# PFLeget/treegp

Hardware: AMD Instinct MI355X
Metric: GP solve+predict throughput, 2-D AnisotropicRBF N=65536 (higher is better)
Workload: dtype f64

## Files before the change

include/tgp.h:

```cpp
#ifndef TGP_H
#define TGP_H

#include <stdint.h>

#ifdef __cplusplus
extern "C" {
#endif

typedef struct tgp_ctx tgp_ctx;
typedef struct tgp_factor tgp_factor;

enum {
    TGP_RBF = 0,
    TGP_ARBF = 1,
    TGP_VK = 2,
    TGP_AVK = 3
};

typedef struct {
    int32_t kind;
    int32_t _pad;
    double amp;
    double a, b, c;
    double ell;
// ... 202 lines not shown
int tgp_d_kbuild_lower(tgp_ctx *ctx, const tgp_kernel *k, const double *d_X, int64_t n,
                       const double *d_yerr, double *d_A);
int tgp_d_potrf(tgp_ctx *ctx, double *d_A, int64_t Np, double *d_W);
int tgp_d_potrs(tgp_ctx *ctx, const double *d_A, const double *d_W, int64_t Np, double *d_b);
int tgp_d_potrs_multi(tgp_ctx *ctx, const double *d_A, const double *d_W, int64_t Np, double *d_B, int nrhs);
int tgp_d_unpack_lower(tgp_ctx *ctx, const double *d_A, int64_t Np, int64_t n, double *out);
int tgp_factor_device(tgp_ctx *ctx, const tgp_factor *f, const double **d_A, const double **d_W, int64_t *Np);
int tgp_set_stream(tgp_ctx *ctx, void *hip_stream);
int tgp_reset_stream(tgp_ctx *ctx);
int tgp_set_side_stream(tgp_ctx *ctx, void *hip_stream);
int64_t tgp_dist_panel_rows(int64_t p, int64_t Np, int G, int g);
int64_t tgp_dist_panel_off(int64_t p, int64_t Np, int G, int g);
int64_t tgp_dist_local_elems(int64_t Np, int G, int g);
int tgp_dd_kbuild(tgp_ctx *ctx, const tgp_kernel *k, const double *d_X, int64_t n, const double *d_yerr,
                  double *d_Aloc, const int64_t *d_loff, int G, int g);
int tgp_dd_factor_diag(tgp_ctx *ctx, double *d_Aloc, const int64_t *h_loff, int64_t Np, int kpanel, int G, int g,
                       double *d_W, double *d_bcast);
int tgp_dd_trsm(tgp_ctx *ctx, double *d_Aloc, const int64_t *h_loff, int64_t Np, int kpanel, int G, int g,
                double *d_W, const double *d_bcast);
int tgp_dd_update(tgp_ctx *ctx, double *d_Aloc, const int64_t *d_loff, int64_t Np, int kpanel, int G, int g,
                  const double *d_gathered, int cmax, int col_lo, int col_hi);
int tgp_dd_update2(tgp_ctx *ctx, double *d_Aloc, const int64_t *d_loff, int64_t Np, int kpanel, int G, int g,
                   const double *d_gathered0, int cmax0, const double *d_gathered1, int cmax1, int col_lo,
                   int col_hi);
int tgp_dd_update_group(tgp_ctx *ctx, double *d_Aloc, const int64_t *d_loff, int64_t Np, int kpanel, int G, int g,
                        int nseg, const double *const *d_gathered, const int *cmax, int col_lo, int col_hi);
int tgp_dd_strip_left(tgp_ctx *ctx, double *d_Aloc, const int64_t *h_loff, const int64_t *d_loff, int64_t Np, int kgroup, int b,
                      int G, int g, const double *d_ext);
int tgp_dd_queue_reset(tgp_ctx *ctx);
int tgp_dd_set_exclusive(tgp_ctx *ctx, int on);
int tgp_dd_update_group_queued(tgp_ctx *ctx, double *d_Aloc, const int64_t *d_loff, int64_t Np, int kpanel, int G, int g,
                               int nseg, const double *const *d_gathered, const int *cmax, int col_lo, int col_hi, int nres);
int tgp_dd_update_group_fused(tgp_ctx *ctx, double *d_Aloc, const int64_t *d_loff, int64_t Np, int kpanel, int G, int g, int nseg,
                              const double *const *d_gathered, const int *cmax, int head_cols, int nres);
int tgp_dd_wait_head(tgp_ctx *ctx, tgp_ctx *waiter);
int tgp_dd_tail_assemble(tgp_ctx *ctx, const double *d_gathered, int64_t stride, int64_t Np, int k0, int G, double *d_tail);
int tgp_dd_tail_scatter(tgp_ctx *ctx, const double *d_tail, int64_t Np, int k0, int G, int g, double *d_Aloc, const int64_t *d_loff);
int tgp_handoff_mode(tgp_ctx *ctx);
int tgp_dd_keep_panel(tgp_ctx *ctx, double *d_Afull, int64_t Np, int kpanel, int G, const double *d_bcast,
                      const double *d_gathered, int cmax);
int tgp_dd_fwd_diag(tgp_ctx *ctx, const double *d_Aloc, const int64_t *h_loff, int kb, const double *d_W, double *d_yk);
int tgp_dd_fwd_update(tgp_ctx *ctx, const double *d_Aloc, const int64_t *h_loff, int64_t Np, int kb, int G, int g,
                      const double *d_zk, double *d_yloc);
int tgp_dd_bwd_partial(tgp_ctx *ctx, const double *d_Aloc, const int64_t *h_loff, int64_t Np, int kb, int G, int g,
                       const double *d_aloc, double *d_s);
int tgp_dd_bwd_diag(tgp_ctx *ctx, const double *d_Aloc, const int64_t *h_loff, int kb, const double *d_W, double *d_ak,
                    const double *d_s );
int tgp_dd_logdet_local(tgp_ctx *ctx, const double *d_Aloc, const int64_t *d_loff, int64_t Np, int64_t n, int G, int g,
                        double *d_out);
int tgp_dd_info(tgp_ctx *ctx, int reset);

int tgp_debug_syrk_loop(tgp_ctx *ctx, double *d_A, int64_t Np, int reps, double *ms_per_launch,
                        double *flops_per_launch);
int tgp_debug_tilemap(int64_t T, int32_t *ti, int32_t *tj, int64_t cap);

#ifdef __cplusplus
}
#endif
#endif
```

treegp_amd/_lib.py:

```python
import ctypes as C
import os
import threading

import numpy as np

_HERE = os.path.dirname(os.path.abspath(__file__))
LIB_PATH = os.environ.get("TGP_LIB_PATH") or os.path.join(_HERE, "csrc", "libtgp.so")

TGP_RBF, TGP_ARBF, TGP_VK, TGP_AVK = 0, 1, 2, 3
NTIMINGS = 12


class TgpKernel(C.Structure):
    _fields_ = [("kind", C.c_int32), ("_pad", C.c_int32), ("amp", C.c_double), ("a", C.c_double),
                ("b", C.c_double), ("c", C.c_double), ("ell", C.c_double)]


TGP_SUM_MAX = 4


class TgpKernelSum(C.Structure):
    _fields_ = [("nterms", C.c_int32), ("_pad", C.c_int32), ("term", TgpKernel * TGP_SUM_MAX)]


# ... 43 lines not shown
    "tgp_d_gp_predict": (C.c_int, [_vp, C.POINTER(TgpKernel), _vp, _i64, _vp, _vp, _i64, _vp]),
    "tgp_d_gp_predict_grad": (C.c_int, [_vp, C.POINTER(TgpKernel), _vp, _i64, _vp, _vp, _i64, _vp]),
    "tgp_panel_off": (_i64, [_i64, _i64]),
    "tgp_panel_elems": (_i64, [_i64]),
    "tgp_padded_n": (_i64, [_i64]),
    "tgp_d_kbuild_lower": (C.c_int, [_vp, C.POINTER(TgpKernel), _vp, _i64, _vp, _vp]),
    "tgp_d_potrf": (C.c_int, [_vp, _vp, _i64, _vp]),
    "tgp_d_potrs": (C.c_int, [_vp, _vp, _vp, _i64, _vp]),
    "tgp_d_potrs_multi": (C.c_int, [_vp, _vp, _vp, _i64, _vp, C.c_int]),
    "tgp_gp_solve_dense": (C.c_int, [_vp, _vp, _i64, _vp, _vp, _vp, _dp, _dp, C.POINTER(_vp)]),
    "tgp_d_gp_solve_dense": (C.c_int, [_vp, _vp, _i64, _vp, _vp, _vp, _dp, _dp, C.POINTER(_vp)]),
    "tgp_factor_solve": (C.c_int, [_vp, _vp, _vp, C.c_int, _vp]),
    "tgp_factor_lmul": (C.c_int, [_vp, _vp, _vp, C.c_int, _vp]),
    "tgp_factor_inv_diag": (C.c_int, [_vp, _vp, _vp]),
    "tgp_factor_inv_blocks": (C.c_int, [_vp, _vp, _vp, _i64, _vp]),
    "tgp_gp_solve_batch": (C.c_int, [_vp, C.c_int, _vp, _vp, _i64, _vp, _vp, _vp, _vp, _vp, _vp, _vp]),
    "tgp_gp_solve_grad_batch": (C.c_int, [_vp, C.c_int, _vp, _vp, _i64, _vp, _vp, _vp, _vp, _vp, _vp, _vp]),
    "tgp_gp_loo_batch": (C.c_int, [_vp, C.c_int, _vp, _vp, _i64, _vp, _vp, _vp, _vp, _vp, _vp, _vp, _vp]),
    "tgp_gp_posterior_batch": (C.c_int, [_vp, C.c_int, _vp, _vp, _i64, _vp, _vp, _vp, _vp, _i64, _vp, C.c_int, _vp, _vp, _vp, _vp, _vp]),
    "tgp_gp_predict_cov_dense": (C.c_int, [_vp, _vp, _vp, _vp, _i64, _vp]),
    "tgp_gp_predict_var": (C.c_int, [_vp, _vp, C.POINTER(TgpKernel), _vp, _i64, _vp, _i64, _vp]),
    "tgp_gp_predict_var_dense": (C.c_int, [_vp, _vp, _vp, _vp, _i64, _vp]),
    "tgp_gp_loglik_grad": (C.c_int, [_vp, _vp, C.POINTER(TgpKernel), _vp, _i64, _vp, _vp]),
    "tgp_d_gp_solve_grad": (C.c_int, [_vp, C.POINTER(TgpKernel), _vp, _i64, _vp, _vp, _dp, _dp, _vp]),
    "tgp_gp_loglik_grad_any": (C.c_int, [_vp, _vp, C.POINTER(TgpKernel), _vp, _i64, _vp, _vp]),
    "tgp_d_gp_solve_grad_any": (C.c_int, [_vp, C.POINTER(TgpKernel), _vp, _i64, _vp, _vp, _dp, _dp, _vp]),
    "tgp_gp_solve_grad_batch_any": (C.c_int, [_vp, C.c_int, _vp, _vp, _i64, _vp, _vp, _vp, _vp, _vp, _vp, _vp]),
    "tgp_kernel_matrix_sum": (C.c_int, [_vp, C.POINTER(TgpKernelSum), _vp, _i64, _vp, _i64, _vp]),
    "tgp_d_kbuild_lower_sum": (C.c_int, [_vp, C.POINTER(TgpKernelSum), _vp, _i64, _vp, _vp]),
    "tgp_gp_solve_sum": (C.c_int, [_vp, C.POINTER(TgpKernelSum), _vp, _i64, _vp, _vp, _vp, _dp, _dp, C.POINTER(_vp)]),
    "tgp_gp_predict_sum": (C.c_int, [_vp, C.POINTER(TgpKernelSum), _vp, _i64, _vp, _vp, _i64, _vp]),
    "tgp_gp_predict_grad_sum": (C.c_int, [_vp, C.POINTER(TgpKernelSum), _vp, _i64, _vp, _vp, _i64, _vp]),
    "tgp_gp_predict_cov_sum": (C.c_int, [_vp, _vp, C.POINTER(TgpKernelSum), _vp, _i64, _vp, _i64, _vp]),
    "tgp_gp_predict_var_sum": (C.c_int, [_vp, _vp, C.POINTER(TgpKernelSum), _vp, _i64, _vp, _i64, _vp]),
    "tgp_gp_loglik_grad_sum": (C.c_int, [_vp, _vp, C.POINTER(TgpKernelSum), _vp, _i64, _vp, _vp]),
    "tgp_gp_fisher": (C.c_int, [_vp, _vp, C.POINTER(TgpKernel), _vp, _i64, _vp]),
    "tgp_gp_fisher_sum": (C.c_int, [_vp, _vp, C.POINTER(TgpKernelSum), _vp, _i64, _vp]),
    "tgp_gp_solve_batch_sum": (C.c_int, [_vp, C.c_int, C.POINTER(TgpKernelSum), _vp, _i64, _vp, _vp, _vp, _vp, _vp, _vp, _vp]),
    "tgp_gp_posterior_batch_sum": (C.c_int, [_vp, C.c_int, C.POINTER(TgpKernelSum), _vp, _i64, _vp, _vp, _vp, _vp, _i64, _vp, C.c_int,
                                             _vp, _vp, _vp, _vp, _vp]),
    "tgp_gp_loo_batch_sum": (C.c_int, [_vp, C.c_int, C.POINTER(TgpKernelSum), _vp, _i64, _vp, _vp, _vp, _vp, _vp, _vp, _vp, _vp]),
    "tgp_gp_solve_grad_batch_sum": (C.c_int, [_vp, C.c_int, C.POINTER(TgpKernelSum), _vp, _i64, _vp, _vp, _vp, _vp, _vp, _vp, _vp]),
    "tgp_kbuild_batch_sum": (C.c_int, [_vp, C.c_int, C.POINTER(TgpKernelSum), _vp, _i64, _vp, _vp, _vp]),
    "tgp_kernel_matrix3": (C.c_int, [_vp, C.POINTER(TgpKernel3), _vp, _i64, _vp, _i64, _vp]),
    "tgp_d_kbuild_lower3": (C.c_int, [_vp, C.POINTER(TgpKernel3), _vp, _i64, _vp, _vp]),
    "tgp_gp_solve3": (C.c_int, [_vp, C.POINTER(TgpKernel3), _vp, _i64, _vp, _vp, _vp, _dp, _dp, C.POINTER(_vp)]),
    "tgp_gp_predict3": (C.c_int, [_vp, C.POINTER(TgpKernel3), _vp, _i64, _vp, _vp, _i64, _vp]),
    "tgp_gp_predict_grad3": (C.c_int, [_vp, C.POINTER(TgpKernel3), _vp, _i64, _vp, _vp, _i64, _vp]),
    "tgp_gp_predict_cov3": (C.c_int, [_vp, _vp, C.POINTER(TgpKernel3), _vp, _i64, _vp, _i64, _vp]),
    "tgp_gp_predict_var3": (C.c_int, [_vp, _vp, C.POINTER(TgpKernel3), _vp, _i64, _vp, _i64, _vp]),
    "tgp_d_unpack_lower":(C.c_int, [_vp, _vp, _i64, _i64, _vp]),
    "tgp_factor_device": (C.c_int, [_vp, _vp, C.POINTER(_vp), C.POINTER(_vp), C.POINTER(_i64)]),
    "tgp_debug_syrk_loop": (C.c_int, [_vp, _vp, _i64, C.c_int, _dp, _dp]),
    "tgp_debug_tilemap": (C.c_int, [_i64, _vp, _vp, _i64]),
    "tgp_set_stream": (C.c_int, [_vp, _vp]),
    "tgp_reset_stream": (C.c_int, [_vp]),
    "tgp_set_side_stream": (C.c_int, [_vp, _vp]),
    "tgp_dist_panel_rows": (_i64, [_i64, _i64, C.c_int, C.c_int]),
    "tgp_dist_panel_off": (_i64, [_i64, _i64, C.c_int, C.c_int]),
    "tgp_dist_local_elems": (_i64, [_i64, C.c_int, C.c_int]),
    "tgp_dd_kbuild": (C.c_int, [_vp, C.POINTER(TgpKernel), _vp, _i64, _vp, _vp, _vp, C.c_int, C.c_int]),
    "tgp_dd_factor_diag": (C.c_int, [_vp, _vp, _vp, _i64, C.c_int, C.c_int, C.c_int, _vp, _vp]),
    "tgp_dd_trsm": (C.c_int, [_vp, _vp, _vp, _i64, C.c_int, C.c_int, C.c_int, _vp, _vp]),
    "tgp_dd_update": (C.c_int, [_vp, _vp, _vp, _i64, C.c_int, C.c_int, C.c_int, _vp, C.c_int, C.c_int, C.c_int]),
    "tgp_dd_update2": (C.c_int, [_vp, _vp, _vp, _i64, C.c_int, C.c_int, C.c_int, _vp, C.c_int, _vp, C.c_int, C.c_int, C.c_int]),
    "tgp_dd_update_group": (C.c_int, [_vp, _vp, _vp, _i64, C.c_int, C.c_int, C.c_int, C.c_int, _vp, _vp, C.c_int, C.c_int]),
    "tgp_dd_strip_left": (C.c_int, [_vp, _vp, _vp, _vp, _i64, C.c_int, C.c_int, C.c_int, C.c_int, _vp]),
    "tgp_dd_update_group_queued": (C.c_int, [_vp, _vp, _vp, _i64, C.c_int, C.c_int, C.c_int, C.c_int, _vp, _vp, C.c_int, C.c_int, C.c_int]),
    "tgp_dd_update_group_fused": (C.c_int, [_vp, _vp, _vp, _i64, C.c_int, C.c_int, C.c_int, C.c_int, _vp, _vp, C.c_int, C.c_int]),
    "tgp_dd_wait_head": (C.c_int, [_vp, _vp]),
    "tgp_handoff_mode": (C.c_int, [_vp]),
    "tgp_dd_tail_assemble": (C.c_int, [_vp, _vp, _i64, _i64, C.c_int, C.c_int, _vp]),
    "tgp_dd_tail_scatter": (C.c_int, [_vp, _vp, _i64, C.c_int, C.c_int, C.c_int, _vp, _vp]),
    "tgp_dd_queue_reset": (C.c_int, [_vp]),
    "tgp_dd_set_exclusive": (C.c_int, [_vp, C.c_int]),
    "tgp_dd_keep_panel": (C.c_int, [_vp, _vp, _i64, C.c_int, C.c_int, _vp, _vp, C.c_int]),
    "tgp_dd_fwd_diag": (C.c_int, [_vp, _vp, _vp, C.c_int, _vp, _vp]),
    "tgp_dd_fwd_update": (C.c_int, [_vp, _vp, _vp, _i64, C.c_int, C.c_int, C.c_int, _vp, _vp]),
    "tgp_dd_bwd_partial": (C.c_int, [_vp, _vp, _vp, _i64, C.c_int, C.c_int, C.c_int, _vp, _vp]),
    "tgp_dd_bwd_diag": (C.c_int, [_vp, _vp, _vp, C.c_int, _vp, _vp, _vp]),
    "tgp_dd_logdet_local": (C.c_int, [_vp, _vp, _vp, _i64, _i64, C.c_int, C.c_int, _vp]),
    "tgp_dd_info": (C.c_int, [_vp, C.c_int]),
}

_lib = None
_ctx = {}
_lock = threading.Lock()


def _share_hip_runtime_with_torch():
    import sys
    if "torch" in sys.modules or os.environ.get("TGP_SYSTEM_HIP") == "1":
        return
    try:
        import importlib.util
        spec = importlib.util.find_spec("torch")
        if spec is None or not spec.origin:
            return
        cand = os.path.join(os.path.dirname(spec.origin), "lib", "libamdhip64.so")
        if os.path.exists(cand):
            C.CDLL(cand, mode=C.RTLD_GLOBAL)
            if os.environ.get("TGP_VERBOSE"):
                print("treegp_amd: using torch's HIP runtime %s (one HIP runtime per process)" % cand, file=sys.stderr)
    except Exception:
        pass

# ... 123 lines not shown
```

treegp_amd/csrc/chol.hip:

```cpp
#include "tgp_internal.h"

#include "gemm_tile.h"
#include "potrf128.h"

#ifdef TGP_POTRF_STAMPS
__device__ unsigned long long tgp_gemm_stamps[1024 * 4];
__device__ int tgp_gemm_stamp_grid = 43;
__device__ unsigned long long tgp_queue_stamps[1024 * 4];
__device__ int tgp_queue_stamp_T = 40;
__device__ unsigned long long tgp_mid_stamps[25 * 8];
__device__ int tgp_mid_stamp_base = 5120;
#define TGP_MID_STAMP(i)                                                                                   \
    do {                                                                                                   \
        if (threadIdx.x == 0 && base == tgp_mid_stamp_base && blockIdx.x < 25) tgp_mid_stamps[blockIdx.x * 8 + (i)] = __builtin_amdgcn_s_memrealtime(); \
    } while (0)
#else
#define TGP_MID_STAMP(i) ((void)0)
#endif

namespace {
template <int MODE, int LDB>
__global__ __launch_bounds__(256, 2) void gemm_col_kernel(const double *A, const double *B, double *C) {
    const int64_t t = blockIdx.x;
    TGP_CHAIN_PRIO();
#ifdef TGP_POTRF_STAMPS
    const unsigned long long t_in = __builtin_amdgcn_s_memrealtime();
#endif
    gemm_tile_128<MODE, LDB, TGP_TB>(A + t * 128 * TGP_PW, B, C + t * 128 * TGP_PW);
#ifdef TGP_POTRF_STAMPS
    if (MODE == 0 && threadIdx.x == 0 && (int)gridDim.x == tgp_gemm_stamp_grid) {
        tgp_gemm_stamps[blockIdx.x * 4 + 0] = t_in;
        tgp_gemm_stamps[blockIdx.x * 4 + 1] = __builtin_amdgcn_s_memrealtime();
        tgp_gemm_stamps[blockIdx.x * 4 + 2] = (__builtin_amdgcn_s_getreg(20 | (0 << 6) | (3 << 11)) << 8) | __builtin_amdgcn_s_getreg(4 | (8 << 6) | (7 << 11));
    }
#endif
}

template <int MODE, int LDB>
__global__ __launch_bounds__(256) void gemm_col_small_kernel(const double *A, const double *B, double *C) {
    const int64_t o = (int64_t)blockIdx.x * 16 * TGP_PW;
    TGP_CHAIN_PRIO();
    nt_slice_tile<MODE, TGP_TB, 1>(nt_slice_lds_storage(), A + o, TGP_PW, B, LDB, C + o, TGP_PW, nullptr, nullptr);
}
__device__ __forceinline__ void keep_w_share(double *__restrict__ keep, const double *__restrict__ W0) {
    if (!keep) return;
    constexpr int n2 = TGP_TB * TGP_TB;
    const int per = (n2 + (int)gridDim.x - 1) / (int)gridDim.x;
    const int lo = (int)blockIdx.x * per, hi = lo + per < n2 ? lo + per : n2;
    for (int i = lo + (int)threadIdx.x; i < hi; i += 256)
        reinterpret_cast<double2 *>(keep)[i] = reinterpret_cast<const double2 *>(W0)[i];
}
__global__ __launch_bounds__(256, 2) void panel_tall_kernel(double *rows0, const double *W0, const double *L10, const double *W1,
                                                            double *keep) {
    double *rows = rows0 + (int64_t)blockIdx.x * 128 * TGP_PW;
    TGP_CHAIN_PRIO();
    keep_w_share(keep, W0);
    gemm_tile_128<0, TGP_TB, TGP_TB>(rows, W0, rows);
    __syncthreads();
    gemm_tile_128<1, TGP_PW, TGP_TB>(rows, L10, rows + TGP_TB);
    __syncthreads();
    gemm_tile_128<0, TGP_TB, TGP_TB>(rows + TGP_TB, W1, rows + TGP_TB);
}

__global__ __launch_bounds__(256) void panel_tall_small_kernel(double *rows0, const double *W0, const double *L10, const double *W1,
                                                               double *keep) {
    double *rows = rows0 + (int64_t)blockIdx.x * 16 * TGP_PW;
    TGP_CHAIN_PRIO();
    keep_w_share(keep, W0);
    double *lds = nt_slice_lds_storage();
    nt_slice_tile<0, TGP_TB, 1>(lds, rows, TGP_PW, W0, TGP_TB, rows, TGP_PW, nullptr, nullptr);
    asm volatile("s_waitcnt vmcnt(0)" ::: "memory");
    __syncthreads();
    nt_slice_tile<1, TGP_TB, 1>(lds, rows, TGP_PW, L10, TGP_PW, rows + TGP_TB, TGP_PW, nullptr, nullptr);
    asm volatile("s_waitcnt vmcnt(0)" ::: "memory");
    __syncthreads();
    nt_slice_tile<0, TGP_TB, 1>(lds, rows + TGP_TB, TGP_PW, W1, TGP_TB, rows + TGP_TB, TGP_PW, nullptr, nullptr);
}

__global__ __launch_bounds__(256, 2) void diag_mid_kernel(double *R1, const double *W0) {
    TGP_CHAIN_PRIO();
    gemm_tile_128<0, TGP_TB, TGP_TB>(R1, W0, R1);
    __syncthreads();
    gemm_tile_128<1, TGP_PW, TGP_TB>(R1, R1, R1 + TGP_TB);
}

constexpr unsigned long long PANEL_SPIN_TICKS = 5000000ull;
constexpr int PANEL_SYNC_WORDS = 16;
__device__ __forceinline__ void panel_publish(unsigned *counter) {
    asm volatile("s_waitcnt vmcnt(0)" ::: "memory");
    __syncthreads();
    if (threadIdx.x == 0) {
        __builtin_amdgcn_fence(__ATOMIC_RELEASE, "agent");
        __hip_atomic_fetch_add(counter, 1u, __ATOMIC_RELAXED, __HIP_MEMORY_SCOPE_AGENT);
    }
}
__device__ __forceinline__ bool panel_wait(unsigned *sync, int which, unsigned target, int *info) {
    __shared__ int s_ok;
    if (threadIdx.x == 0) {
        int ok = 1;
        const unsigned long long t0 = __builtin_amdgcn_s_memrealtime();
        unsigned it = 0;
        while (__hip_atomic_load(sync + which, __ATOMIC_RELAXED, __HIP_MEMORY_SCOPE_AGENT) < target) {
            __builtin_amdgcn_s_sleep(1);
            if ((++it & 63u) == 0u) {
                const bool late = __builtin_amdgcn_s_memrealtime() - t0 > PANEL_SPIN_TICKS;
                if (late || __hip_atomic_load(sync + 2, __ATOMIC_RELAXED, __HIP_MEMORY_SCOPE_AGENT) != 0u) {
                    __hip_atomic_store(sync + 2, 1u, __ATOMIC_RELAXED, __HIP_MEMORY_SCOPE_AGENT);
                    if (late) __hip_atomic_store(info, -7, __ATOMIC_RELAXED, __HIP_MEMORY_SCOPE_AGENT);
                    ok = 0;
                    break;
                }
            }
        }
        __builtin_amdgcn_fence(__ATOMIC_ACQUIRE, "agent");
// ... 360 lines not shown

template <int NSEG>
__global__ __launch_bounds__(256, 2) void syrk_distn_queue_kernel(double *Aloc, const int64_t *__restrict__ loff, int kpanel, int G,
                                                                  int g, DistSegs<NSEG> S, int col_lo, int ncol, int nrows, DistMap M,
                                                                  unsigned slots_per_class, int nres, unsigned *__restrict__ queue) {
    __shared__ unsigned s_slot;
    const unsigned xcd = blockIdx.x & 7;
    if (threadIdx.x == 0) {
        const unsigned hw = __builtin_amdgcn_s_getreg(4 | (8 << 6) | (7 << 11));
        const unsigned xcc = __builtin_amdgcn_s_getreg(20 | (0 << 6) | (3 << 11)) & 7;
        const unsigned key = hw + 1;
        unsigned *claims = queue + 8 + TGP_QUEUE_MAXRES * (4 * xcc + ((hw >> 5) & 3));
        unsigned leave = 0;
        for (int r = 0; r < nres && !leave; ++r) {
            const unsigned prev = atomicCAS(&claims[r], 0u, key);
            leave = (prev == 0u || prev == key) ? 1u : 0u;
        }
        if (leave && atomicAdd(&queue[TGP_QUEUE_LEAVE + xcd], 1u) >= 8u * (unsigned)nres + 8u) leave = 0u;
        s_slot = leave;
    }
    __syncthreads();
    const bool leave = s_slot != 0u;
    __syncthreads();
    if (leave) return;
    for (;;) {
        if (threadIdx.x == 0) s_slot = atomicAdd(&queue[xcd], 1u);
        __syncthreads();
        const unsigned n = s_slot;
        __syncthreads();
        if (n >= slots_per_class) break;
        syrk_distn_tile<NSEG>(((int64_t)n << 3) | xcd, Aloc, loff, kpanel, G, g, S, col_lo, ncol, nrows, M);
        __syncthreads();
    }
}

inline void run_potrf128(hipStream_t st, double *A, int lda, double *W, int *info, int base, bool exclusive = false, bool solo = false) {
    constexpr unsigned image = potrf_v2::POTRF_LDS_BYTES, full = 128 * 1024;
    static const bool attr_ok = [] {
        return hipFuncSetAttribute((const void *)potrf_v2::potrf128_kernel<true>, hipFuncAttributeMaxDynamicSharedMemorySize, (int)full) == hipSuccess &&
               hipFuncSetAttribute((const void *)potrf_v2::potrf128_solo_kernel, hipFuncAttributeMaxDynamicSharedMemorySize, (int)full) == hipSuccess;
    }();
    (void)attr_ok;
    if (exclusive || solo) potrf_v2::potrf128_solo_kernel<<<1, 256, exclusive ? full : image, st>>>(A, lda, W, info, base);
    else potrf_v2::potrf128_kernel<true><<<1, 256, image, st>>>(A, lda, W, info, base);
}
}

namespace {
__global__ void set_identity128_kernel(double *__restrict__ W) {
    const int t = blockIdx.x * 256 + threadIdx.x;
    W[t] = (t >> 7) == (t & 127) ? 1.0 : 0.0;
}

void factor_panel(hipStream_t st, double *Pk, int64_t mk, double *W0, int *d_info, int base, bool exclusive = false,
                  int64_t n_data = -1, unsigned *mid_sync = nullptr, int cu_budget = 0) {
    double *W1 = W0 + TGP_TB * TGP_TB;
    double *R1 = Pk + (int64_t)TGP_TB * TGP_PW;
    const int r1 = (int)((mk - TGP_TB) / TGP_TB);
    static const int small_rows = [] { const char *e = getenv("TGP_SMALL_ROWS"); return e ? atoi(e) : 80; }();
    const bool solo = cu_budget >= 256 && mid_sync != nullptr;
    run_potrf128(st, Pk, TGP_PW, W0, d_info, base, exclusive, solo);
    if (n_data >= 0 && (int64_t)base + TGP_TB >= n_data && mk == TGP_PW) {
        gemm_col_small_kernel<0, TGP_TB><<<8, 256, 0, st>>>(R1, W0, R1);
        set_identity128_kernel<<<64, 256, 0, st>>>(W1);
        return;
    }
    const int r2 = (int)((mk - TGP_PW) / TGP_TB);
    if (mid_sync) {
        constexpr unsigned pad = 128 * 1024 - potrf_v2::POTRF_LDS_DOUBLES * 8;
        static const bool pad_ok = [] {
            return hipFuncSetAttribute((const void *)panel_mid_kernel<true>, hipFuncAttributeMaxDynamicSharedMemorySize, (int)pad) == hipSuccess &&
                   hipFuncSetAttribute((const void *)panel_mid_kernel<false>, hipFuncAttributeMaxDynamicSharedMemorySize, (int)pad) == hipSuccess;
        }();
        const unsigned dyn = (exclusive && pad_ok) ? pad : 0u;
        if (17 + 8 * r2 <= cu_budget) panel_mid_kernel<true><<<25 + 8 * r2, 256, dyn, st>>>(Pk, W0, W1, d_info, base, mid_sync);
        else panel_mid_kernel<false><<<25 + r2, 256, dyn, st>>>(Pk, W0, W1, d_info, base, mid_sync);
    } else if (cu_budget > 0) {
        double *R2 = Pk + (int64_t)TGP_PW * TGP_PW;
        const bool small = 17 + 8 * r2 <= cu_budget;
        gemm_col_small_kernel<0, TGP_TB><<<8, 256, 0, st>>>(R1, W0, R1);
        if (r2 > 0) {
            if (small) gemm_col_small_kernel<0, TGP_TB><<<r2 * 8, 256, 0, st>>>(R2, W0, R2);
            else gemm_col_kernel<0, TGP_TB><<<r2, 256, 0, st>>>(R2, W0, R2);
        }
        gemm_col_small_kernel<1, TGP_PW><<<8, 256, 0, st>>>(R1, R1, R1 + TGP_TB);
        if (r2 > 0) {
            if (small) gemm_col_small_kernel<1, TGP_PW><<<r2 * 8, 256, 0, st>>>(R2, R1, R2 + TGP_TB);
            else gemm_col_kernel<1, TGP_PW><<<r2, 256, 0, st>>>(R2, R1, R2 + TGP_TB);
        }
        run_potrf128(st, R1 + TGP_TB, TGP_PW, W1, d_info, base + TGP_TB, exclusive, solo);
    } else {
        if (r1 <= small_rows) {
            gemm_col_small_kernel<0, TGP_TB><<<r1 * 8, 256, 0, st>>>(R1, W0, R1);
            gemm_col_small_kernel<1, TGP_PW><<<r1 * 8, 256, 0, st>>>(R1, R1, R1 + TGP_TB);
        } else {
            gemm_col_kernel<0, TGP_TB><<<r1, 256, 0, st>>>(R1, W0, R1);
            gemm_col_kernel<1, TGP_PW><<<r1, 256, 0, st>>>(R1, R1, R1 + TGP_TB);
        }
        run_potrf128(st, R1 + TGP_TB, TGP_PW, W1, d_info, base + TGP_TB, exclusive, solo);
    }
    if (r2 > 0) {
        double *R2 = Pk + (int64_t)TGP_PW * TGP_PW + TGP_TB;
        if (r2 <= small_rows) gemm_col_small_kernel<0, TGP_TB><<<r2 * 8, 256, 0, st>>>(R2, W1, R2);
        else gemm_col_kernel<0, TGP_TB><<<r2, 256, 0, st>>>(R2, W1, R2);
    }
}

inline int diag_full() {
    static const int v = [] { const char *e = getenv("TGP_DIAG_FULL"); return e ? (atoi(e) != 0 ? 1 : 0) : 0; }();
    return v;
}

inline int small_t() {
    static const int v = [] { const char *e = getenv("TGP_SMALL_T"); return e ? atoi(e) : 8; }();
    return v;
}

template <int NSEG>
void launch_syrk(hipStream_t st, double *d_A, int64_t Np, int ob, int T, int strip, const double *P0, const double *P1) {
    if (T <= 0) return;
    static const int strip_small_t = [] { const char *e = getenv("TGP_STRIP_SMALL_T"); return e ? atoi(e) : 16; }();
    if (T <= small_t() || (strip > 0 && T <= strip_small_t)) {
        const int cols = strip == 0 ? T : (strip < T ? strip : T);
        syrk_small_kernel<NSEG><<<dim3((unsigned)(T * 8), (unsigned)cols), 256, 0, st>>>(d_A, Np, ob, T, P0, P1);
        return;
    }
    static const int strip64_t = [] { const char *e = getenv("TGP_STRIP64_T"); return e ? atoi(e) : 128; }();
    static const int strip32_t = [] { const char *e = getenv("TGP_STRIP32_T"); return e ? atoi(e) : 64; }();
    if (strip > 0 && T <= strip32_t) {
        syrk_strip32_kernel<NSEG><<<(unsigned)((int64_t)4 * T * strip), 256, 0, st>>>(d_A, Np, ob, T, strip, P0, P1);
        return;
    }
    if (strip > 0 && T <= strip64_t) {
        syrk_strip64_kernel<NSEG><<<(unsigned)((int64_t)2 * T * strip), 256, 0, st>>>(d_A, Np, ob, T, strip, P0, P1);
        return;
    }
    const unsigned gs = strip == 0 ? (unsigned)tilemap_grid(T) : (unsigned)((int64_t)T * strip);
    syrk_dtv_kernel<NSEG><<<gs, 256, 0, st>>>(d_A, Np, ob, T, strip, P0, P1, diag_full());
}

int queued_nres(int T) {
    static const int queue_res = [] { const char *e = getenv("TGP_QUEUE_RES"); return e ? atoi(e) : 0; }();
    if (queue_res > 0) return queue_res > TGP_QUEUE_MAXRES ? TGP_QUEUE_MAXRES : queue_res;
    static const int t1 = [] { const char *e = getenv("TGP_QUEUE_T1"); return e ? atoi(e) : 42; }();
    static const int t2 = [] { const char *e = getenv("TGP_QUEUE_T2"); return e ? atoi(e) : 26; }();
    return T >= t1 ? 1 : (T >= t2 ? 2 : 3);
}
void launch_syrk2_queued(tgp_ctx *ctx, hipStream_t st, double *d_A, int64_t Np, int ob, int T, const double *P0, const double *P1,
                         int nqueue) {
    const int nres = queued_nres(T);
    static const int half_env = [] { const char *e = getenv("TGP_QUEUE_HALF"); return e ? atoi(e) : -1; }();
    const unsigned slots = (unsigned)(tilemap_grid(T) / 8);
    unsigned nhalf = half_env >= 0 ? (unsigned)half_env : (unsigned)(512 - 64 * nres) / 8u;
    if (nhalf > slots) nhalf = slots;
    static const int steal = [] { const char *e = getenv("TGP_QUEUE_STEAL"); return e ? atoi(e) : 1; }();
    syrk_dtv_queue_kernel<2><<<512 + 8, 256, 0, st>>>(d_A, Np, ob, T, slots + nhalf, slots - nhalf, nres,
// ... 207 lines not shown
            }
        }
    }
    TGP_HIP(hipGetLastError());
    TGP_HIP(hipMemcpyAsync(ctx->h_info, ctx->d_info, sizeof(int), hipMemcpyDeviceToHost, st));
    ctx->timings[6] = nlaunch;
    ctx->timings[7] = flops;
    ctx->timings[5] = 0.0;
    if (defer_info && !prof) return 0;
    TGP_HIP(hipStreamSynchronize(st));
    if (prof) {
        double tot = 0.0;
        for (int i = 0; i < nlaunch; ++i) {
            float ms = 0.f;
            TGP_HIP(hipEventElapsedTime(&ms, ctx->prof_events[2 * i], ctx->prof_events[2 * i + 1]));
            tot += ms;
        }
        ctx->timings[5] = tot;
    }
    return tgp_potrf_info_rc(ctx, *ctx->h_info);
}

int tgp_potrf_info_rc(tgp_ctx *ctx, int info) {
    if (info >= 0) return info;
    ctx->err = "Cholesky: an in-kernel hand-off timed out (panel_mid_kernel waited 50 ms for workgroups of its own launch); "
               "the factor is incomplete -- TGP_PANEL_MID=0 selects the schedule without in-kernel waits";
    return TGP_RC_HANDOFF;
}

int launch_factor_diag256(tgp_ctx *ctx, double *blk, double *W0, double *W1, int base, bool latency) {
    hipStream_t st = ctx->stream;
    double *R1 = blk + (int64_t)TGP_TB * TGP_PW;
    const bool excl = ctx->chain_exclusive != 0;
    run_potrf128(st, blk, TGP_PW, W0, ctx->d_info, base, excl);
    if (latency) {
        gemm_col_small_kernel<0, TGP_TB><<<8, 256, 0, st>>>(R1, W0, R1);
        gemm_col_small_kernel<1, TGP_PW><<<8, 256, 0, st>>>(R1, R1, R1 + TGP_TB);
    } else {
        diag_mid_kernel<<<1, 256, 0, st>>>(R1, W0);
    }
    run_potrf128(st, R1 + TGP_TB, TGP_PW, W1, ctx->d_info, base + TGP_TB, excl);
    TGP_HIP(hipGetLastError());
    return 0;
}

int launch_trsm_rows(tgp_ctx *ctx, double *rows, int ntiles, const double *Lkk, const double *W0, const double *W1, double *keepW) {
    if (ntiles <= 0) {
        if (keepW) TGP_HIP(hipMemcpyAsync(keepW, W0, (size_t)2 * TGP_TB * TGP_TB * 8, hipMemcpyDeviceToDevice, ctx->stream));
        return 0;
    }
    constexpr int small_max = 24;
    if (ntiles <= small_max)
        panel_tall_small_kernel<<<ntiles * 8, 256, 0, ctx->stream>>>(rows, W0, Lkk + (int64_t)TGP_TB * TGP_PW, W1, keepW);
    else
        panel_tall_kernel<<<ntiles, 256, 0, ctx->stream>>>(rows, W0, Lkk + (int64_t)TGP_TB * TGP_PW, W1, keepW);
    TGP_HIP(hipGetLastError());
    return 0;
}

template <int NSEG>
static void launch_distn(hipStream_t st, unsigned grid, double *d_Aloc, const int64_t *d_loff, int kpanel, int G, int g,
                         const double *const *P, const int *cmax, int col_lo, int ncol, int nrows, const DistMap &M, int nres,
                         unsigned *queue, const double *const *PB) {
    DistSegs<NSEG> S;
    for (int s = 0; s < NSEG; ++s) {
        S.P[s] = P[s];
        S.PB[s] = PB ? PB[s] : P[s];
        S.cmax[s] = cmax[s];
        S.frg[s] = (int)dist_first_round(kpanel + s + 1, g, G);
    }
    if (nres > 0 && queue)
        syrk_distn_queue_kernel<NSEG><<<512 + 8, 256, 0, st>>>(d_Aloc, d_loff, kpanel, G, g, S, col_lo, ncol, nrows, M, grid / 8, nres, queue);
    else
        syrk_distn_kernel<NSEG><<<grid, 256, 0, st>>>(d_Aloc, d_loff, kpanel, G, g, S, col_lo, ncol, nrows, M);
}

int launch_syrk_distn(tgp_ctx *ctx, double *d_Aloc, const int64_t *d_loff, int64_t Np, int kpanel, int G, int g, int nseg,
                      const double *const *d_P, const int *cmax, int col_lo, int col_hi, int queue_nres, int head_cols,
                      const double *const *d_PB) {
    TGP_ARG(nseg >= 1 && nseg <= 4 && head_cols >= 0);
    const int64_t nB = Np / TGP_PW;
    const int64_t nloc = dist_panel_blocks(kpanel + nseg, nB, g, G);
    const int64_t ncol_all = 2 * (nB - kpanel - nseg);
    if (col_hi < 0 || col_hi > ncol_all) col_hi = (int)ncol_all;
    if (col_lo < 0) col_lo = 0;
    const int64_t ncol = (int64_t)col_hi - col_lo;
    hipStream_t st = ctx->stream;
    DistMap M;
    M.nhead = M.head_cols = M.whole = M.head_half = 0;
    M.half_from = 1 << 30;
    constexpr int half_max = 256;
    if (head_cols > 0) {
        hipError_t e = hipSuccess;
        M.hs.seq = tgp_next_seq(ctx, TGP_FLAG_HEAD, &e);
        TGP_HIP(e);
        M.hs.flag = ctx->d_flags + 16 * TGP_FLAG_HEAD;
        M.hs.done = ctx->d_flags + 16 * TGP_FLAG_HEAD_COUNT;
    }
    if (nloc <= 0 || ncol <= 0) {
        if (head_cols > 0) TGP_HIP(tgp_signal_value(ctx, st, TGP_FLAG_HEAD, M.hs.seq));
        return 0;
    }
    const int nrows = (int)(2 * nloc);
    const int64_t s0 = kpanel + nseg, qfb = dist_first_round(s0, g, G);
    M.qfb = (int)qfb;
    M.ginv = G == 1 ? 0u : (unsigned)((((uint64_t)1) << 32) / (uint64_t)G) + 1u;
    TGP_ARG(nB < 65536 && G >= 1);
    unsigned grid = 0;
    if (head_cols == 0 && ncol <= 8 && queue_nres == 0) {
// ... 118 lines not shown
```

treegp_amd/csrc/gemm_tile.h:

```cpp
#pragma once
#include "tgp_internal.h"

typedef double d4 __attribute__((ext_vector_type(4)));

constexpr int KB = 16;

template <int LSV, bool PRE>
struct TileCfg {
    static constexpr int LS = LSV;
    static constexpr bool PRELOAD = PRE;
};
using TileDefault = TileCfg<17, true>;

using v2u = __attribute__((ext_vector_type(2))) unsigned;
using v4u = __attribute__((ext_vector_type(4))) unsigned;
__device__ __forceinline__ __amdgpu_buffer_rsrc_t tile_rsrc(const double *p, int bytes) {
    return __builtin_amdgcn_make_buffer_rsrc(const_cast<double *>(p), 0, bytes, 0x00020000);
}
__device__ __forceinline__ double buf_ld1(__amdgpu_buffer_rsrc_t r, int voff, int soff) {
    return __builtin_bit_cast(double, __builtin_amdgcn_raw_buffer_load_b64(r, voff, soff, 0));
}
__device__ __forceinline__ double2 buf_ld2(__amdgpu_buffer_rsrc_t r, int voff, int soff) {
    return __builtin_bit_cast(double2, __builtin_amdgcn_raw_buffer_load_b128(r, voff, soff, 0));
}
// ... 115 lines not shown
#pragma unroll
        for (int k4 = 0; k4 < KB / 4; ++k4) {
            double af[4], bf[4];
#pragma unroll
            for (int m = 0; m < 4; ++m) af[m] = As[fa + m * 16 * LS + k4 * 4];
#pragma unroll
            for (int n = 0; n < 4; ++n) bf[n] = Bs[fb + n * 16 * LS + k4 * 4];
#pragma unroll
            for (int m = 0; m < 4; ++m)
#pragma unroll
                for (int n = 0; n < 4; ++n)
                    acc[m][n] = __builtin_amdgcn_mfma_f64_16x16x4f64(af[m], bf[n], acc[m][n], 0, 0, 0);
        }
        __builtin_amdgcn_sched_barrier(0);
        if (more) {
#pragma unroll
            for (int s = 0; s < 4; ++s) {
                lds_put2<LS>(&lds[buf ^ 1][0][(srow + 32 * s) * LS + kp], ra[s]);
                lds_put2<LS>(&lds[buf ^ 1][1][(srow + 32 * s) * LS + kp], rb[s]);
            }
        }
        __syncthreads();
    }

#pragma unroll
    for (int m = 0; m < 4; ++m) {
        if constexpr (MODE == 1 && !PRELOAD) {
            double old[4][4];
#pragma unroll
            for (int n = 0; n < 4; ++n)
#pragma unroll
                for (int r = 0; r < 4; ++r) old[n][r] = buf_ld1(rc_dst, vc, ((m * 16 + 4 * r) * LDC + n * 16) * 8);
#pragma unroll
            for (int n = 0; n < 4; ++n)
#pragma unroll
                for (int r = 0; r < 4; ++r)
                    buf_st1(old[n][r] - acc[m][n][r], rc_dst, vc, ((m * 16 + 4 * r) * LDC + n * 16) * 8);
        } else {
#pragma unroll
            for (int n = 0; n < 4; ++n)
#pragma unroll
                for (int r = 0; r < 4; ++r)
                    buf_st1((PRELOAD || MODE == 2) ? -acc[m][n][r] : acc[m][n][r], rc_dst, vc, ((m * 16 + 4 * r) * LDC + n * 16) * 8);
        }
    }
}

template <int MODE, int LDB, int KDEPTH, typename CFG = TileDefault, int NSEG = 1>
__device__ __forceinline__ void gemm_tile_128(const double *a_ptr, const double *b_ptr, double *c_ptr,
                                              const double *a1_ptr = nullptr, const double *b1_ptr = nullptr, int nseg_rt = 1,
                                              int64_t seg_stride_a = 0, int64_t seg_stride_b = 0) {
    gemm_tile_128_at<MODE, LDB, KDEPTH, CFG, NSEG>(tile128_lds_storage<CFG::LS>(), a_ptr, b_ptr, c_ptr, a1_ptr, b1_ptr, nseg_rt,
                                                   seg_stride_a, seg_stride_b);
}


constexpr int DTV_LSB = 18;
__device__ __forceinline__ double *dtv_lds_storage() {
    __shared__ __attribute__((aligned(16))) double lds[2 * 128 * DTV_LSB];
    return lds;
}

template <int NW, int KDEPTH, int NSEG, int MT = 2>
__device__ __forceinline__ void gemm_tile_dtv(const double *a_ptr, const double *b_ptr, double *c_ptr,
                                              const double *a1_ptr, const double *b1_ptr, int nseg_rt = 1,
                                              int64_t seg_stride_a = 0, int64_t seg_stride_b = 0) {
    constexpr int LD = TGP_PW;
    constexpr int LSB = DTV_LSB;
    constexpr int BPT = 16 / NW;
    constexpr int BROWS = 8 * NW;
    double (*ldsB)[128 * LSB] = reinterpret_cast<double (*)[128 * LSB]>(dtv_lds_storage());

    const int tid = threadIdx.x;
    const int lane = tid & 63;
    const int w = __builtin_amdgcn_readfirstlane(tid >> 6);
    const int l15 = lane & 15, l4 = lane >> 4;

    const __amdgpu_buffer_rsrc_t ra0 = tile_rsrc(a_ptr, 16 * MT * NW * LD * 8);
    const __amdgpu_buffer_rsrc_t rb0 = tile_rsrc(b_ptr, 128 * LD * 8);
    const __amdgpu_buffer_rsrc_t ra1 = tile_rsrc(NSEG > 1 ? a1_ptr : a_ptr, 16 * MT * NW * LD * 8);
    const __amdgpu_buffer_rsrc_t rb1 = tile_rsrc(NSEG > 1 ? b1_ptr : b_ptr, 128 * LD * 8);
    const __amdgpu_buffer_rsrc_t rc = tile_rsrc(c_ptr, 16 * MT * NW * LD * 8);
    const int va = ((16 * MT * w + l15) * LD + 2 * l4) * 8;
    const int srow = tid >> 3, kp = (tid & 7) * 2;
    const int vb = (srow * LD + kp) * 8;
    const int vc = ((16 * MT * w + l4) * LD + l15) * 8;
    const int fb = l15 * LSB + 2 * l4;

    double2 areg[2][MT][2];
    double2 rbst[BPT];
    auto load_a = [&](double2 (&dst)[MT][2], __amdgpu_buffer_rsrc_t src, int k0) {
#pragma unroll
        for (int m = 0; m < MT; ++m)
#pragma unroll
            for (int h = 0; h < 2; ++h) dst[m][h] = buf_ld2(src, va, (m * 16 * LD + k0 + 8 * h) * 8);
    };
    auto load_b = [&](__amdgpu_buffer_rsrc_t src, int k0) {
#pragma unroll
        for (int s = 0; s < BPT; ++s) rbst[s] = buf_ld2(src, vb, (s * BROWS * LD + k0) * 8);
    };
    auto store_b = [&](int buf) {
#pragma unroll
        for (int s = 0; s < BPT; ++s) *reinterpret_cast<double2 *>(&ldsB[buf][(srow + BROWS * s) * LSB + kp]) = rbst[s];
    };
    load_a(areg[0], ra0, 0);
    load_b(rb0, 0);
// ... 601 lines not shown
```

Before: 246,600.

## Skip zero upper-triangle products in panel TRSM tiles and add fused panel kernel

Adds a triangular-aware 128x128 GEMM tile that multiplies only the chunks where the inverse-triangular W block is nonzero (chunk <= column block). Work is dealt so both wave columns get equal counts. panel_tall_kernel now uses this triangular tile by default, cutting MFMA work in the two W-multiply steps roughly in half. An optional fused single-pass panel_rows_kernel (env TGP_PANEL_PASSES=1) and a debug entry point are also added. The risk is correctness if W is not strictly lower-triangular in the expected orientation, plus per-wave branching overhead.

```diff
diff --git a/include/tgp.h b/include/tgp.h
--- a/include/tgp.h
+++ b/include/tgp.h
@@ -278,6 +278,8 @@
 
 int tgp_debug_syrk_loop(tgp_ctx *ctx, double *d_A, int64_t Np, int reps, double *ms_per_launch,
                         double *flops_per_launch);
+int tgp_debug_panel_solve(tgp_ctx *ctx, double *d_rows, int row_tiles, const double *d_W0, const double *d_L10,
+                          const double *d_W1, int passes);
 int tgp_debug_tilemap(int64_t T, int32_t *ti, int32_t *tj, int64_t cap);
 
 #ifdef __cplusplus
diff --git a/treegp_amd/_lib.py b/treegp_amd/_lib.py
--- a/treegp_amd/_lib.py
+++ b/treegp_amd/_lib.py
@@ -119,6 +119,7 @@
     "tgp_d_unpack_lower":(C.c_int, [_vp, _vp, _i64, _i64, _vp]),
     "tgp_factor_device": (C.c_int, [_vp, _vp, C.POINTER(_vp), C.POINTER(_vp), C.POINTER(_i64)]),
     "tgp_debug_syrk_loop": (C.c_int, [_vp, _vp, _i64, C.c_int, _dp, _dp]),
+    "tgp_debug_panel_solve": (C.c_int, [_vp, _vp, C.c_int, _vp, _vp, _vp, C.c_int]),
     "tgp_debug_tilemap": (C.c_int, [_i64, _vp, _vp, _i64]),
     "tgp_set_stream": (C.c_int, [_vp, _vp]),
     "tgp_reset_stream": (C.c_int, [_vp]),
diff --git a/treegp_amd/csrc/chol.hip b/treegp_amd/csrc/chol.hip
--- a/treegp_amd/csrc/chol.hip
+++ b/treegp_amd/csrc/chol.hip
@@ -50,16 +50,38 @@
     for (int i = lo + (int)threadIdx.x; i < hi; i += 256)
         reinterpret_cast<double2 *>(keep)[i] = reinterpret_cast<const double2 *>(W0)[i];
 }
+template <bool TRI>
+__device__ __forceinline__ void panel_rows_body(double *rows, const double *W0, const double *L10, const double *W1) {
+    if constexpr (TRI) gemm_tile_128_tri(rows, W0, rows);
+    else gemm_tile_128<0, TGP_TB, TGP_TB>(rows, W0, rows);
+    __syncthreads();
+    gemm_tile_128<1, TGP_PW, TGP_TB>(rows, L10, rows + TGP_TB);
+    __syncthreads();
+    if constexpr (TRI) gemm_tile_128_tri(rows + TGP_TB, W1, rows + TGP_TB);
+    else gemm_tile_128<0, TGP_TB, TGP_TB>(rows + TGP_TB, W1, rows + TGP_TB);
+}
+template <bool TRI>
 __global__ __launch_bounds__(256, 2) void panel_tall_kernel(double *rows0, const double *W0, const double *L10, const double *W1,
                                                             double *keep) {
     double *rows = rows0 + (int64_t)blockIdx.x * 128 * TGP_PW;
     TGP_CHAIN_PRIO();
     keep_w_share(keep, W0);
-    gemm_tile_128<0, TGP_TB, TGP_TB>(rows, W0, rows);
-    __syncthreads();
-    gemm_tile_128<1, TGP_PW, TGP_TB>(rows, L10, rows + TGP_TB);
-    __syncthreads();
-    gemm_tile_128<0, TGP_TB, TGP_TB>(rows + TGP_TB, W1, rows + TGP_TB);
+    panel_rows_body<TRI>(rows, W0, L10, W1);
+}
+__global__ __launch_bounds__(256, 2) void panel_rows_kernel(double *rows0, const double *W0, const double *L10, const double *W1) {
+    double *rows = rows0 + (int64_t)blockIdx.x * 128 * TGP_PW;
+    TGP_CHAIN_PRIO();
+#ifdef TGP_POTRF_STAMPS
+    const unsigned long long t_in = __builtin_amdgcn_s_memrealtime();
+#endif
+    panel_rows_body<true>(rows, W0, L10, W1);
+#ifdef TGP_POTRF_STAMPS
+    if (threadIdx.x == 0 && (int)gridDim.x == tgp_gemm_stamp_grid && blockIdx.x < 1024) {
+        tgp_gemm_stamps[blockIdx.x * 4 + 0] = t_in;
+        tgp_gemm_stamps[blockIdx.x * 4 + 1] = __builtin_amdgcn_s_memrealtime();
+        tgp_gemm_stamps[blockIdx.x * 4 + 2] = (__builtin_amdgcn_s_getreg(20 | (0 << 6) | (3 << 11)) << 8) | __builtin_amdgcn_s_getreg(4 | (8 << 6) | (7 << 11));
+    }
+#endif
 }
 
 __global__ __launch_bounds__(256) void panel_tall_small_kernel(double *rows0, const double *W0, const double *L10, const double *W1,
@@ -526,6 +548,11 @@
     W[t] = (t >> 7) == (t & 127) ? 1.0 : 0.0;
 }
 
+inline int panel_passes() {
+    static const int v = [] { const char *e = getenv("TGP_PANEL_PASSES"); const int n = e ? atoi(e) : 0; return n == 1 || n == 3 ? n : 0; }();
+    return v;
+}
+
 void factor_panel(hipStream_t st, double *Pk, int64_t mk, double *W0, int *d_info, int base, bool exclusive = false,
                   int64_t n_data = -1, unsigned *mid_sync = nullptr, int cu_budget = 0) {
     double *W1 = W0 + TGP_TB * TGP_TB;
@@ -540,6 +567,7 @@
         return;
     }
     const int r2 = (int)((mk - TGP_PW) / TGP_TB);
+    bool fused = false;
     if (mid_sync) {
         constexpr unsigned pad = 128 * 1024 - potrf_v2::POTRF_LDS_DOUBLES * 8;
         static const bool pad_ok = [] {
@@ -552,30 +580,34 @@
     } else if (cu_budget > 0) {
         double *R2 = Pk + (int64_t)TGP_PW * TGP_PW;
         const bool small = 17 + 8 * r2 <= cu_budget;
+        fused = panel_passes() == 1 && !small && r2 > small_rows;
         gemm_col_small_kernel<0, TGP_TB><<<8, 256, 0, st>>>(R1, W0, R1);
-        if (r2 > 0) {
+        if (r2 > 0 && !fused) {
             if (small) gemm_col_small_kernel<0, TGP_TB><<<r2 * 8, 256, 0, st>>>(R2, W0, R2);
             else gemm_col_kernel<0, TGP_TB><<<r2, 256, 0, st>>>(R2, W0, R2);
         }
         gemm_col_small_kernel<1, TGP_PW><<<8, 256, 0, st>>>(R1, R1, R1 + TGP_TB);
-        if (r2 > 0) {
+        if (r2 > 0 && !fused) {
             if (small) gemm_col_small_kernel<1, TGP_PW><<<r2 * 8, 256, 0, st>>>(R2, R1, R2 + TGP_TB);
             else gemm_col_kernel<1, TGP_PW><<<r2, 256, 0, st>>>(R2, R1, R2 + TGP_TB);
         }
         run_potrf128(st, R1 + TGP_TB, TGP_PW, W1, d_info, base + TGP_TB, exclusive, solo);
     } else {
+        fused = panel_passes() == 1 && r1 > small_rows && r2 > small_rows;
         if (r1 <= small_rows) {
             gemm_col_small_kernel<0, TGP_TB><<<r1 * 8, 256, 0, st>>>(R1, W0, R1);
             gemm_col_small_kernel<1, TGP_PW><<<r1 * 8, 256, 0, st>>>(R1, R1, R1 + TGP_TB);
         } else {
-            gemm_col_kernel<0, TGP_TB><<<r1, 256, 0, st>>>(R1, W0, R1);
-            gemm_col_kernel<1, TGP_PW><<<r1, 256, 0, st>>>(R1, R1, R1 + TGP_TB);
+            const int tiles = fused ? 1 : r1;
+            gemm_col_kernel<0, TGP_TB><<<tiles, 256, 0, st>>>(R1, W0, R1);
+            gemm_col_kernel<1, TGP_PW><<<tiles, 256, 0, st>>>(R1, R1, R1 + TGP_TB);
         }
         run_potrf128(st, R1 + TGP_TB, TGP_PW, W1, d_info, base + TGP_TB, exclusive, solo);
     }
     if (r2 > 0) {
         double *R2 = Pk + (int64_t)TGP_PW * TGP_PW + TGP_TB;
-        if (r2 <= small_rows) gemm_col_small_kernel<0, TGP_TB><<<r2 * 8, 256, 0, st>>>(R2, W1, R2);
+        if (fused) panel_rows_kernel<<<r2, 256, 0, st>>>(Pk + (int64_t)TGP_PW * TGP_PW, W0, R1, W1);
+        else if (r2 <= small_rows) gemm_col_small_kernel<0, TGP_TB><<<r2 * 8, 256, 0, st>>>(R2, W1, R2);
         else gemm_col_kernel<0, TGP_TB><<<r2, 256, 0, st>>>(R2, W1, R2);
     }
 }
@@ -889,9 +921,28 @@
     constexpr int small_max = 24;
     if (ntiles <= small_max)
         panel_tall_small_kernel<<<ntiles * 8, 256, 0, ctx->stream>>>(rows, W0, Lkk + (int64_t)TGP_TB * TGP_PW, W1, keepW);
+    else if (panel_passes() == 3)
+        panel_tall_kernel<false><<<ntiles, 256, 0, ctx->stream>>>(rows, W0, Lkk + (int64_t)TGP_TB * TGP_PW, W1, keepW);
     else
-        panel_tall_kernel<<<ntiles, 256, 0, ctx->stream>>>(rows, W0, Lkk + (int64_t)TGP_TB * TGP_PW, W1, keepW);
+        panel_tall_kernel<true><<<ntiles, 256, 0, ctx->stream>>>(rows, W0, Lkk + (int64_t)TGP_TB * TGP_PW, W1, keepW);
     TGP_HIP(hipGetLastError());
+    return 0;
+}
+
+int tgp_debug_panel_solve(tgp_ctx *ctx, double *d_rows, int row_tiles, const double *d_W0, const double *d_L10, const double *d_W1,
+                          int passes) {
+    TGP_ARG(d_rows && d_W0 && d_L10 && d_W1 && row_tiles > 0 && row_tiles <= 65535 && (passes == 1 || passes == 3));
+    TGP_HIP(hipSetDevice(ctx->device));
+    hipStream_t st = ctx->stream;
+    if (passes == 1) {
+        panel_rows_kernel<<<row_tiles, 256, 0, st>>>(d_rows, d_W0, d_L10, d_W1);
+    } else {
+        gemm_col_kernel<0, TGP_TB><<<row_tiles, 256, 0, st>>>(d_rows, d_W0, d_rows);
+        gemm_col_kernel<1, TGP_PW><<<row_tiles, 256, 0, st>>>(d_rows, d_L10, d_rows + TGP_TB);
+        gemm_col_kernel<0, TGP_TB><<<row_tiles, 256, 0, st>>>(d_rows + TGP_TB, d_W1, d_rows + TGP_TB);
+    }
+    TGP_HIP(hipGetLastError());
+    TGP_HIP(hipStreamSynchronize(st));
     return 0;
 }
 
diff --git a/treegp_amd/csrc/gemm_tile.h b/treegp_amd/csrc/gemm_tile.h
--- a/treegp_amd/csrc/gemm_tile.h
+++ b/treegp_amd/csrc/gemm_tile.h
@@ -191,6 +191,137 @@
                                               int64_t seg_stride_a = 0, int64_t seg_stride_b = 0) {
     gemm_tile_128_at<MODE, LDB, KDEPTH, CFG, NSEG>(tile128_lds_storage<CFG::LS>(), a_ptr, b_ptr, c_ptr, a1_ptr, b1_ptr, nseg_rt,
                                                    seg_stride_a, seg_stride_b);
+}
+
+
+constexpr int tri_deal_jb(int wc, int n) { return n == 0 ? wc : n == 1 ? 3 - wc : n == 2 ? 4 + wc : 7 - wc; }
+constexpr bool tri_deal_runs(int wc, int n, int chunk) { return chunk <= tri_deal_jb(wc, n); }
+constexpr int tri_deal_count(int wc) {
+    int cnt = 0;
+    for (int n = 0; n < 4; ++n)
+        for (int c = 0; c < 8; ++c) cnt += tri_deal_runs(wc, n, c) ? 1 : 0;
+    return cnt;
+}
+constexpr unsigned long long tri_deal_cover() {
+    unsigned long long mask = 0;
+    for (int wc = 0; wc < 2; ++wc)
+        for (int n = 0; n < 4; ++n)
+            for (int c = 0; c < 8; ++c) {
+                if (!tri_deal_runs(wc, n, c)) continue;
+                const unsigned long long bit = 1ull << (8 * tri_deal_jb(wc, n) + c);
+                if (mask & bit) return ~0ull;
+                mask |= bit;
+            }
+    return mask;
+}
+constexpr unsigned long long tri_needed_products() {
+    unsigned long long mask = 0;
+    for (int jb = 0; jb < 8; ++jb)
+        for (int c = 0; c <= jb; ++c) mask |= 1ull << (8 * jb + c);
+    return mask;
+}
+static_assert(tri_deal_count(0) == 18 && tri_deal_count(1) == 18, "both wave columns run 18 block-chunks per m-tile");
+static_assert(tri_deal_jb(0, 0) + tri_deal_jb(0, 3) == 7 && tri_deal_jb(0, 1) + tri_deal_jb(0, 2) == 7 &&
+              tri_deal_jb(1, 0) + tri_deal_jb(1, 3) == 7 && tri_deal_jb(1, 1) + tri_deal_jb(1, 2) == 7, "column blocks jb and 7 - jb together");
+static_assert(tri_deal_cover() == tri_needed_products(), "the deal runs exactly the products chunk <= jb, each once");
+
+template <int WC, typename CFG>
+__device__ __forceinline__ void tile128_tri_wave(double *lds_base, const double *a_ptr, const double *b_ptr, double *c_ptr) {
+    constexpr int LDA = TGP_PW, LDC = TGP_PW, LDB = TGP_TB;
+    constexpr int LS = CFG::LS;
+    constexpr int NCH = TGP_TB / KB;
+    static_assert(NCH == 8, "eight 16-deep chunks, eight 16-column blocks");
+    double (*lds)[2][128 * LS] = reinterpret_cast<double (*)[2][128 * LS]>(lds_base);
+
+    const int tid = threadIdx.x;
+    const int lane = tid & 63;
+    const int wr = __builtin_amdgcn_readfirstlane(tid >> 7);
+    const int l15 = lane & 15, l4 = lane >> 4;
+
+    const int srow = tid >> 3;
+    const int kp = (tid & 7) * 2;
+    const __amdgpu_buffer_rsrc_t ra_src = tile_rsrc(a_ptr, 128 * LDA * 8);
+    const __amdgpu_buffer_rsrc_t rb_src = tile_rsrc(b_ptr, 128 * LDB * 8);
+    const __amdgpu_buffer_rsrc_t rc_dst = tile_rsrc(c_ptr, 128 * LDC * 8);
+    const int va = (srow * LDA + kp) * 8, vb = (srow * LDB + kp) * 8;
+
+    double2 ra[4], rb[4];
+#pragma unroll
+    for (int s = 0; s < 4; ++s) {
+        ra[s] = buf_ld2(ra_src, va, s * 32 * LDA * 8);
+        rb[s] = buf_ld2(rb_src, vb, s * 32 * LDB * 8);
+    }
+    const int vc = ((wr * 64 + l4) * LDC + l15) * 8;
+    d4 acc[4][4];
+#pragma unroll
+    for (int m = 0; m < 4; ++m)
+#pragma unroll
+        for (int n = 0; n < 4; ++n) acc[m][n] = (d4){0.0, 0.0, 0.0, 0.0};
+#pragma unroll
+    for (int s = 0; s < 4; ++s) {
+        lds_put2<LS>(&lds[0][0][(srow + 32 * s) * LS + kp], ra[s]);
+        lds_put2<LS>(&lds[0][1][(srow + 32 * s) * LS + kp], rb[s]);
+    }
+    __syncthreads();
+
+    const int fa = (wr * 64 + l15) * LS + l4;
+    const int fb = l15 * LS + l4;
+#pragma unroll
+    for (int c = 0; c < NCH; ++c) {
+        const int buf = c & 1;
+        const bool more = (c + 1 < NCH);
+        if (more) {
+#pragma unroll
+            for (int s = 0; s < 4; ++s) {
+                ra[s] = buf_ld2(ra_src, va, (s * 32 * LDA + (c + 1) * KB) * 8);
+                rb[s] = buf_ld2(rb_src, vb, (s * 32 * LDB + (c + 1) * KB) * 8);
+            }
+        }
+        const double *As = lds[buf][0];
+        const double *Bs = lds[buf][1];
+#pragma unroll
+        for (int k4 = 0; k4 < KB / 4; ++k4) {
+            double af[4], bf[4];
+#pragma unroll
+            for (int m = 0; m < 4; ++m) af[m] = As[fa + m * 16 * LS + k4 * 4];
+#pragma unroll
+            for (int n = 0; n < 4; ++n)
+                if (tri_deal_runs(WC, n, c)) bf[n] = Bs[fb + tri_deal_jb(WC, n) * 16 * LS + k4 * 4];
+#pragma unroll
+            for (int m = 0; m < 4; ++m)
+#pragma unroll
+                for (int n = 0; n < 4; ++n)
+                    if (tri_deal_runs(WC, n, c)) acc[m][n] = __builtin_amdgcn_mfma_f64_16x16x4f64(af[m], bf[n], acc[m][n], 0, 0, 0);
+        }
+        __builtin_amdgcn_sched_barrier(0);
+        if (more) {
+#pragma unroll
+            for (int s = 0; s < 4; ++s) {
+                lds_put2<LS>(&lds[buf ^ 1][0][(srow + 32 * s) * LS + kp], ra[s]);
+                lds_put2<LS>(&lds[buf ^ 1][1][(srow + 32 * s) * LS + kp], rb[s]);
+            }
+        }
+        __syncthreads();
+    }
+
+#pragma unroll
+    for (int m = 0; m < 4; ++m)
+#pragma unroll
+        for (int n = 0; n < 4; ++n)
+#pragma unroll
+            for (int r = 0; r < 4; ++r)
+                buf_st1(acc[m][n][r], rc_dst, vc, ((m * 16 + 4 * r) * LDC + tri_deal_jb(WC, n) * 16) * 8);
+}
+
+template <typename CFG = TileDefault>
+__device__ __forceinline__ void gemm_tile_128_tri_at(double *lds_base, const double *a_ptr, const double *w_ptr, double *c_ptr) {
+    const int wc = __builtin_amdgcn_readfirstlane((threadIdx.x >> 6) & 1);
+    if (wc == 0) tile128_tri_wave<0, CFG>(lds_base, a_ptr, w_ptr, c_ptr);
+    else tile128_tri_wave<1, CFG>(lds_base, a_ptr, w_ptr, c_ptr);
+}
+template <typename CFG = TileDefault>
+__device__ __forceinline__ void gemm_tile_128_tri(const double *a_ptr, const double *w_ptr, double *c_ptr) {
+    gemm_tile_128_tri_at<CFG>(tile128_lds_storage<CFG::LS>(), a_ptr, w_ptr, c_ptr);
 }
 
 
```

After: 246,600, median of 2. About the same (+0.0%).
